# ikt-luh/Unified-Point-Cloud-Compression

Measured on AMD Instinct MI355X. Metric: points/sec encode+decode, longdress vox10, 1 GPU; bpp & D1-PSNR parity, higher is better.
Workload: dtype f32

## Files before the change

### include/pcc_hip.h

```cpp
#ifndef PCC_HIP_H
#define PCC_HIP_H

#include <stddef.h>
#include <stdint.h>

#ifdef __cplusplus
extern "C" {
#endif

#define PCC_OK 0
#define PCC_EINVAL (-1)
#define PCC_EHIP (-2)
#define PCC_EWS (-3)

#define PCC_ACT_NONE 0
#define PCC_ACT_RELU 1
#define PCC_ACT_LEAKY 2

#define PCC_MAP_HDR_INTS 512
#define PCC_MAP_MAX_SEG 8

int pcc_version(void);
const char* pcc_last_error(void);
int pcc_device_info(int* h_cu_count, char* h_arch, int h_arch_len);
// ... 30 lines not shown
int pcc_coords_expand_csr(const int64_t* keys, int64_t n, int32_t kernel_size, int32_t ts_out,
                          const int32_t* h_lattice, int64_t* out_keys, int64_t* d_count, int32_t* pair_ids,
                          int32_t* first, void* ws, size_t ws_bytes, void* stream);

int64_t pcc_map_nbr_elems(int64_t n_out, int32_t kernel_size, int32_t stride, int32_t transposed);
size_t pcc_map_ws_bytes(int64_t n_out);
int pcc_kernel_map_build(const int64_t* in_keys, int64_t n_in, const int64_t* out_keys, int64_t n_out,
                         int32_t kernel_size, int32_t step, int32_t stride, int32_t transposed,
                         int32_t* hdr, int32_t* nbr, int32_t* rows ,
                         int64_t* d_pairs, const uint64_t* grid_bits , const int32_t* grid_rank,
                         const int32_t* h_grid, void* ws, size_t ws_bytes, void* stream);

int64_t pcc_grid_words(const int32_t* h_grid);
size_t pcc_grid_ws_bytes(int64_t words);
int pcc_grid_build(const int64_t* keys, int64_t n, const int32_t* h_grid, uint64_t* bits ,
                   int32_t* rank , void* ws, size_t ws_bytes, void* stream);
int pcc_coords_stride_grid(const int64_t* keys, int64_t n, const int64_t* d_n, const int32_t* h_grid, uint64_t* bits,
                           int32_t* rank, int64_t* out_keys, int64_t* d_count, void* ws, size_t ws_bytes, void* stream);
int pcc_keys_canonicalize_grid(const int64_t* keys, int64_t n, const int32_t* h_grid, uint64_t* bits, int32_t* rank,
                               int64_t* out_keys, int32_t* first_user, int64_t* d_count, void* ws, size_t ws_bytes,
                               void* stream);
int pcc_coords_expand_grid(const int64_t* keys, int64_t n, int32_t kernel_size, const int32_t* h_out, uint64_t* bits,
                           int32_t* rank, int64_t* out_keys, int64_t* d_count, void* ws, size_t ws_bytes, void* stream);
size_t pcc_convt_rows_int_ws_bytes(int64_t pairs, int32_t K);
int64_t pcc_convt_rows_t_elems(int64_t pairs, int32_t K, int32_t cout);
int pcc_convt_fwd_rows(const float* feat_in, int64_t n_in, int32_t cin, const float* packed_w, const float* bias,
                       int32_t K, int32_t cout, const int32_t* first, const int32_t* pair_ids, int64_t n_out,
                       int64_t pairs, float* T, float* out, int32_t act, float slope, void* int_ws, size_t int_ws_bytes,
                       int32_t arith , int32_t* d_guard , void* stream);
int pcc_map_from_csr(const int32_t* first, const int32_t* pair_ids, int64_t n_out, int32_t kernel_size, int32_t* hdr,
                     int32_t* nbr, void* stream);
size_t pcc_expand_grid_csr_ws_bytes(int64_t n_out);
int pcc_coords_expand_grid_csr(const int64_t* out_keys, int64_t n_out, int32_t kernel_size, int32_t ts_out,
                               const uint64_t* in_bits, const int32_t* in_rank, const int32_t* h_in, int64_t n_in,
                               int32_t* first, int32_t* pair_ids, int64_t* d_total, void* ws, size_t ws_bytes, void* stream);
int64_t pcc_expand_grid_csr_slot_elems(int64_t n_out, int32_t kernel_size);
int pcc_coords_expand_grid_csr_slots(const int64_t* out_keys, int64_t n_out, int32_t kernel_size, int32_t ts_out,
                                     const uint64_t* in_bits, const int32_t* in_rank, const int32_t* h_in, int64_t n_in,
                                     int32_t* first, int32_t* pair_ids, int32_t* wg_end, int64_t* d_total , int32_t zk,
                                     void* stream);
int pcc_coords_expand_grid_csr_zk(const int64_t* out_keys, int64_t n_out, int32_t kernel_size, int32_t ts_out,
                               const uint64_t* in_bits, const int32_t* in_rank, const int32_t* h_in, int64_t n_in,
                               int32_t* first, int32_t* pair_ids, int64_t* d_total, void* ws, size_t ws_bytes, void* stream);
int pcc_map_to_dense(const int32_t* hdr, const int32_t* nbr, const int32_t* rows, int64_t n_out,
                     int32_t K, int32_t* dense, void* stream);

// ... 231 lines not shown
```

### unified_point_cloud_compression_amd/csrc/pcc_keys.hip

```cpp
#include <stdarg.h>
#include <stdio.h>
#include <string.h>

#include "pcc_common.h"

static thread_local char g_err[512] = "";

void pcc_set_error(const char* fmt, ...) {
  va_list ap;
  va_start(ap, fmt);
  vsnprintf(g_err, sizeof(g_err), fmt, ap);
  va_end(ap);
}

extern "C" const char* pcc_last_error(void) { return g_err; }
extern "C" int pcc_version(void) { return 100; }

extern "C" int pcc_device_info(int* h_cu_count, char* h_arch, int h_arch_len) {
  int dev = 0;
  PCC_CHECK_HIP(hipGetDevice(&dev));
  hipDeviceProp_t p;
  PCC_CHECK_HIP(hipGetDeviceProperties(&p, dev));
  if (h_cu_count) *h_cu_count = p.multiProcessorCount;
  if (h_arch && h_arch_len > 0) {
// ... 666 lines not shown
    }
  }
#pragma unroll
  for (int c = 0; c < 4; ++c) {
    for (int d = 32; d >= 1; d >>= 1) { mn[c] = min(mn[c], __shfl_xor(mn[c], d)); mx[c] = max(mx[c], __shfl_xor(mx[c], d)); }
    if ((threadIdx.x & 63) == 0) { atomicMin(&s_min[c], mn[c]); atomicMax(&s_max[c], mx[c]); }
  }
  __syncthreads();
  if (threadIdx.x < 4) { atomicMin(&out8[threadIdx.x], s_min[threadIdx.x]); atomicMax(&out8[4 + threadIdx.x], s_max[threadIdx.x]); }
}

extern "C" int pcc_coords_bounds(const void* coords, int32_t is_float, int64_t n, int32_t* out8, void* stream) {
  hipStream_t s = (hipStream_t)stream;
  PCC_REQUIRE(coords && out8 && n >= 1, "pcc_coords_bounds: bad arguments");
  PCC_CHECK_HIP(hipMemsetAsync(out8, 0x7F, 16, s));
  PCC_CHECK_HIP(hipMemsetAsync(out8 + 4, 0x80, 16, s));
  const unsigned g = (unsigned)(pcc_cdiv(n, 256) < 1024 ? pcc_cdiv(n, 256) : 1024);
  if (is_float) k_coords_bounds<float><<<g, 256, 0, s>>>((const float*)coords, n, out8);
  else k_coords_bounds<int><<<g, 256, 0, s>>>((const int*)coords, n, out8);
  PCC_LAUNCH_CHECK();
  return PCC_OK;
}

__device__ __forceinline__ void intake_block_reduce(int (&v)[9], int* __restrict__ part) {
  __shared__ int s_red[4][9];
#pragma unroll
  for (int c = 0; c < 9; ++c) {
    for (int d = 32; d >= 1; d >>= 1) v[c] = min(v[c], __shfl_xor(v[c], d));
    if ((threadIdx.x & 63) == 0) s_red[threadIdx.x >> 6][c] = v[c];
  }
  __syncthreads();
  if (threadIdx.x < 9) {
    const int c = threadIdx.x;
    part[blockIdx.x * 16 + c] = min(min(s_red[0][c], s_red[1][c]), min(s_red[2][c], s_red[3][c]));
  }
}

__global__ void __launch_bounds__(256) k_frame_intake(const float* __restrict__ pc, long long n, long long* __restrict__ keys,
                                                      float4* __restrict__ feats, int* __restrict__ part) {
  int v[9] = {0, 0x7FFFFFFF, 0x7FFFFFFF, 0x7FFFFFFF, 0, 0x7FFFFFFF, 0x7FFFFFFF, 0x7FFFFFFF, 1};
  for (long long i = (long long)blockIdx.x * 256 + threadIdx.x; i < n; i += (long long)gridDim.x * 256) {
    const float2* r = reinterpret_cast<const float2*>(pc + i * 6);
    const float2 a = r[0], b = r[1], c = r[2];
    const int x = (int)floorf(a.x), y = (int)floorf(a.y), z = (int)floorf(b.x);
    const long long k = pack4(0, x, y, z);
    keys[i] = k;
    feats[i] = make_float4(1.f, b.y, c.x, c.y);
    v[1] = min(v[1], x); v[2] = min(v[2], y); v[3] = min(v[3], z);
    v[5] = min(v[5], -x); v[6] = min(v[6], -y); v[7] = min(v[7], -z);
    if (i > 0) {
      const float* q = pc + (i - 1) * 6;
      if (k <= pack4(0, (int)floorf(q[0]), (int)floorf(q[1]), (int)floorf(q[2]))) v[8] = 0;
    }
  }
  intake_block_reduce(v, part);
}

__global__ void __launch_bounds__(256) k_coords_intake_i32(const int4* __restrict__ c4, long long n, long long* __restrict__ keys,
                                                           int* __restrict__ part) {
  int v[9] = {0x7FFFFFFF, 0x7FFFFFFF, 0x7FFFFFFF, 0x7FFFFFFF, 0x7FFFFFFF, 0x7FFFFFFF, 0x7FFFFFFF, 0x7FFFFFFF, 1};
  for (long long i = (long long)blockIdx.x * 256 + threadIdx.x; i < n; i += (long long)gridDim.x * 256) {
    const int4 c = c4[i];
    const long long k = pack4(c.x, c.y, c.z, c.w);
    keys[i] = k;
    v[0] = min(v[0], c.x); v[1] = min(v[1], c.y); v[2] = min(v[2], c.z); v[3] = min(v[3], c.w);
    v[4] = min(v[4], -c.x); v[5] = min(v[5], -c.y); v[6] = min(v[6], -c.z); v[7] = min(v[7], -c.w);
    if (i > 0) {
      const int4 q = c4[i - 1];
      if (k <= pack4(q.x, q.y, q.z, q.w)) v[8] = 0;
    }
  }
  intake_block_reduce(v, part);
}

__global__ void __launch_bounds__(256) k_intake_reduce(const int* __restrict__ part, int nblk, int* __restrict__ out12) {
  __shared__ int s_red[4][9];
  int v[9];
#pragma unroll
  for (int c = 0; c < 9; ++c) v[c] = 0x7FFFFFFF;
  for (int b = threadIdx.x; b < nblk; b += 256)
#pragma unroll
    for (int c = 0; c < 9; ++c) v[c] = min(v[c], part[b * 16 + c]);
#pragma unroll
  for (int c = 0; c < 9; ++c) {
    for (int d = 32; d >= 1; d >>= 1) v[c] = min(v[c], __shfl_xor(v[c], d));
    if ((threadIdx.x & 63) == 0) s_red[threadIdx.x >> 6][c] = v[c];
  }
  __syncthreads();
  if (threadIdx.x < 9) {
    const int c = threadIdx.x;
    out12[c] = min(min(s_red[0][c], s_red[1][c]), min(s_red[2][c], s_red[3][c]));
  }
}

extern "C" size_t pcc_frame_intake_ws_bytes(void) { return (size_t)1024 * 16 * sizeof(int); }

extern "C" int pcc_frame_intake(const float* pc, int64_t n, int64_t* keys, float* feats, int32_t* out12, void* ws, size_t ws_bytes,
                                void* stream) {
  hipStream_t s = (hipStream_t)stream;
  PCC_REQUIRE(pc && keys && feats && out12 && ws && n >= 1, "pcc_frame_intake: bad arguments");
  PCC_REQUIRE((((uintptr_t)pc & 7) | ((uintptr_t)feats & 15)) == 0, "pcc_frame_intake: the frame must be 8-byte, the features 16-byte aligned");
  if (ws_bytes < pcc_frame_intake_ws_bytes()) { pcc_set_error("pcc_frame_intake: workspace too small"); return PCC_EWS; }
  const unsigned g = (unsigned)(pcc_cdiv(n, 256) < 1024 ? pcc_cdiv(n, 256) : 1024);
  k_frame_intake<<<g, 256, 0, s>>>(pc, n, (long long*)keys, (float4*)feats, (int*)ws);
  k_intake_reduce<<<1, 256, 0, s>>>((const int*)ws, (int)g, out12);
  PCC_LAUNCH_CHECK();
  return PCC_OK;
}

extern "C" int pcc_coords_intake_i32(const int32_t* coords, int64_t n, int64_t* keys, int32_t* out12, void* ws, size_t ws_bytes,
                                     void* stream) {
  hipStream_t s = (hipStream_t)stream;
// ... 53 lines not shown
```

### unified_point_cloud_compression_amd/csrc/pcc_map.hip

```cpp
#include <string.h>

#include "pcc_common.h"

struct SegPlan {
  int nseg;
  int K;
  int listed;
  int k_count[PCC_MAP_MAX_SEG];
  int koff_begin[PCC_MAP_MAX_SEG];
  unsigned char koffs[192];
  unsigned char order[192];
};

__device__ __forceinline__ void write_hdr(const SegPlan& plan, const int* __restrict__ class_begin, int class_stride,
                                          int64_t n_out, int* __restrict__ hdr) {
  {
    const int i = (int)threadIdx.x;
    if (i < plan.K && i < 192) {
      hdr[HDR_KOFFS + i] = plan.listed ? plan.koffs[i] : i;
      hdr[HDR_ORDER + i] = plan.order[i];
    }
  }
  if (threadIdx.x != 0) return;
  hdr[HDR_NSEG] = plan.nseg;
// ... 334 lines not shown
  int* class_begin = (int*)p;           p += 1024;
  void* sort_ws = p;
  dim3 g1((unsigned)pcc_cdiv(n_out, 256));
  k_classify<<<g1, 256, 0, s>>>(out_keys, n_out, ilog2(step), stride, cls);
  PCC_LAUNCH_CHECK();
  PCC_TRY(pcc_sort_keys((const int64_t*)cls, n_out, 0xFFull, (int64_t*)cls_sorted, rows, sort_ws,
                        ws_bytes - (size_t)(p - (char*)ws), s));
  k_class_begin<<<1, 64, 0, s>>>(cls_sorted, n_out, nclass, class_begin);
  PCC_LAUNCH_CHECK();
  k_write_hdr<<<1, 192, 0, s>>>(plan, class_begin, 1, n_out, hdr);
  PCC_LAUNCH_CHECK();
  dim3 gdim((unsigned)pcc_cdiv(n_out, 256), (unsigned)max_class_k(kernel_size, stride));
  k_map_transposed<<<gdim, 256, 0, s>>>(grid, in_keys, (int)n_in, out_keys, n_out, kernel_size, step, hdr, rows, nbr,
                                        block_counts);
  PCC_LAUNCH_CHECK();
  if (d_pairs) {
    k_sum_counts<<<1, 1024, 0, s>>>(block_counts, (int64_t)gdim.x * gdim.y, d_pairs);
    PCC_LAUNCH_CHECK();
  }
  return PCC_OK;
}

static int grid_rank(const unsigned long long* b, int64_t words, int32_t* rank, const int32_t* h, int tsl, int64_t* out_keys,
                     int64_t* d_count, void* ws, size_t ws_bytes, hipStream_t s);
__device__ inline long long grid_cell(const int64_t key, const int lo0, const int lo1, const int lo2, const int d0,
                                      const int d1, const int d2, const int tsl) {
  const int b = (int)(key >> 48);
  const int cx = ((int)((key >> 32) & 0xFFFF) - (int)PCC_BIAS - lo0) >> tsl;
  const int cy = ((int)((key >> 16) & 0xFFFF) - (int)PCC_BIAS - lo1) >> tsl;
  const int cz = ((int)(key & 0xFFFF) - (int)PCC_BIAS - lo2) >> tsl;
  return (((long long)b * d0 + cx) * d1 + cy) * d2 + cz;
}

__global__ void k_grid_bits(const int64_t* __restrict__ keys, int64_t n, int lo0, int lo1, int lo2, int d0, int d1,
                            int d2, int tsl, unsigned long long* __restrict__ bits) {
  const int64_t i = (int64_t)blockIdx.x * blockDim.x + threadIdx.x;
  if (i >= n) return;
  const long long c = grid_cell(keys[i], lo0, lo1, lo2, d0, d1, d2, tsl);
  const long long w = c >> 6;
  if (i > 0 && (grid_cell(keys[i - 1], lo0, lo1, lo2, d0, d1, d2, tsl) >> 6) == w) return;
  unsigned long long acc = 1ull << (c & 63);
  for (int64_t t = i + 1; t < n && t < i + 64; ++t) {
    const long long c2 = grid_cell(keys[t], lo0, lo1, lo2, d0, d1, d2, tsl);
    if ((c2 >> 6) != w) break;
    acc |= 1ull << (c2 & 63);
  }
  bits[w] = acc;
// ... 159 lines not shown
    unsigned long long x = bits[wi];
    if (!x) continue;
    int r = rk_s[li];
    long long cell = wi * 64;
    const int z0 = (int)(cell % d2); cell /= d2;
    const int y0 = (int)(cell % d1); cell /= d1;
    const int x0 = (int)(cell % d0);
    const int b0 = (int)(cell / d0);
    while (x) {
      const int bit = __ffsll((long long)x) - 1;
      x &= x - 1;
      int cz = z0 + bit, cy = y0, cx = x0, b = b0;
      while (cz >= d2) {
        cz -= d2;
        if (++cy == d1) { cy = 0; if (++cx == d0) { cx = 0; ++b; } }
      }
      const int64_t X = (int64_t)(lo0 + (cx << tsl)) + PCC_BIAS, Y = (int64_t)(lo1 + (cy << tsl)) + PCC_BIAS,
                    Z = (int64_t)(lo2 + (cz << tsl)) + PCC_BIAS;
      keys[r++] = ((int64_t)b << 48) | (X << 32) | (Y << 16) | Z;
    }
  }
}

static int grid_rank(const unsigned long long* b, int64_t words, int32_t* rank, const int32_t* h, int tsl, int64_t* out_keys,
                     int64_t* d_count, void* ws, size_t ws_bytes, hipStream_t s) {
  const int64_t nb = pcc_cdiv(words, GR_B);
  if (nb <= GR_SELF_NB && (((uintptr_t)b | (uintptr_t)rank) & 15) == 0) {
    if (out_keys) k_grid_rank_apply<true, true><<<(unsigned)nb, 256, 0, s>>>(b, words, nullptr, rank, h[0], h[1], h[2], h[3], h[4], h[5], tsl, out_keys, d_count);
    else k_grid_rank_apply<false, true><<<(unsigned)nb, 256, 0, s>>>(b, words, nullptr, rank, 0, 0, 0, 1, 1, 1, 0, nullptr, nullptr);
    PCC_LAUNCH_CHECK();
    return PCC_OK;
  }
  if (nb <= GR_DIRECT_NB && ws_bytes >= (size_t)nb * 4 + 256 && (((uintptr_t)b | (uintptr_t)rank) & 15) == 0) {
    int* sums = (int*)ws;
    k_grid_rank_reduce<<<(unsigned)nb, 256, 0, s>>>(b, words, sums);
    k_grid_rank_apply<false><<<(unsigned)nb, 256, 0, s>>>(b, words, sums, rank, 0, 0, 0, 1, 1, 1, 0, nullptr, nullptr);
    PCC_LAUNCH_CHECK();
    if (out_keys) {
      k_grid_enumerate<<<(unsigned)pcc_cdiv(words, 256), 256, 0, s>>>(b, rank, words, h[0], h[1], h[2], h[3], h[4], h[5], tsl, out_keys, d_count);
      PCC_LAUNCH_CHECK();
    }
    return PCC_OK;
  }
  k_grid_popc<<<(unsigned)pcc_cdiv(words, 256), 256, 0, s>>>(b, words, rank);
  PCC_LAUNCH_CHECK();
  PCC_TRY(pcc_scan_exclusive_i32(rank, rank, words, ws, ws_bytes, s));
  if (out_keys) {
    k_grid_enumerate<<<(unsigned)pcc_cdiv(words, 256), 256, 0, s>>>(b, rank, words, h[0], h[1], h[2], h[3], h[4], h[5], tsl, out_keys, d_count);
    PCC_LAUNCH_CHECK();
  }
  return PCC_OK;
}

extern "C" int pcc_coords_stride_grid(const int64_t* keys, int64_t n, const int64_t* d_n, const int32_t* h_grid, uint64_t* bits,
                                      int32_t* rank, int64_t* out_keys, int64_t* d_count, void* ws, size_t ws_bytes,
                                      void* stream) {
  hipStream_t s = (hipStream_t)stream;
  PCC_REQUIRE(h_grid && bits && rank && out_keys && d_count, "pcc_coords_stride_grid: NULL array");
// ... 297 lines not shown

__global__ void k_set_int(int* p, int v) { *p = v; }

extern "C" int pcc_coords_expand_grid(const int64_t* keys, int64_t n, int32_t kernel_size, const int32_t* h_out,
                                      uint64_t* bits, int32_t* rank, int64_t* out_keys, int64_t* d_count, void* ws,
                                      size_t ws_bytes, void* stream) {
  hipStream_t s = (hipStream_t)stream;
  PCC_REQUIRE(keys && h_out && bits && rank && out_keys && d_count && n > 0, "pcc_coords_expand_grid: bad arguments");
  PCC_REQUIRE(kernel_size == 2 || kernel_size == 3 || kernel_size == 5, "pcc_coords_expand_grid: kernel_size %d unsupported", kernel_size);
  const int64_t words = pcc_grid_words(h_out);
  PCC_REQUIRE(words >= 1 && words < (1ll << 31), "pcc_coords_expand_grid: lattice too large (%lld words)", (long long)words);
  const int ts_out = h_out[6];
  PCC_REQUIRE(ts_out >= 1 && (ts_out & (ts_out - 1)) == 0, "pcc_coords_expand_grid: pitch must be a power of two");
  if (ws_bytes < pcc_grid_ws_bytes(words)) { pcc_set_error("pcc_coords_expand_grid: workspace too small"); return PCC_EWS; }
  PCC_CHECK_HIP(hipMemsetAsync(bits, 0, (size_t)words * 8, s));
  const dim3 g((unsigned)pcc_cdiv(n, 256), (unsigned)(kernel_size * kernel_size));
  unsigned long long* b = (unsigned long long*)bits;
  const int tsl = ilog2(ts_out);
  if (kernel_size == 2) k_expand_mark<2><<<g, 256, 0, s>>>(keys, n, ts_out, h_out[0], h_out[1], h_out[2], h_out[3], h_out[4], h_out[5], tsl, b);
  else if (kernel_size == 3) k_expand_mark<3><<<g, 256, 0, s>>>(keys, n, ts_out, h_out[0], h_out[1], h_out[2], h_out[3], h_out[4], h_out[5], tsl, b);
  else k_expand_mark<5><<<g, 256, 0, s>>>(keys, n, ts_out, h_out[0], h_out[1], h_out[2], h_out[3], h_out[4], h_out[5], tsl, b);
  PCC_LAUNCH_CHECK();
  return grid_rank(b, words, rank, h_out, tsl, out_keys, d_count, ws, ws_bytes, s);
}

extern "C" size_t pcc_expand_grid_csr_ws_bytes(int64_t n_out) { return pcc_scan_ws_bytes(n_out + 1) + 256; }

static int expand_grid_csr(const int64_t* out_keys, int64_t n_out, int32_t kernel_size, int32_t ts_out,
                           const uint64_t* in_bits, const int32_t* in_rank, const int32_t* h_in,
                           int64_t n_in, int32_t* first, int32_t* pair_ids, int64_t* d_total, void* ws, size_t ws_bytes, int zk,
                           void* stream);
extern "C" int pcc_coords_expand_grid_csr(const int64_t* out_keys, int64_t n_out, int32_t kernel_size, int32_t ts_out,
                                          const uint64_t* in_bits, const int32_t* in_rank, const int32_t* h_in,
                                          int64_t n_in, int32_t* first, int32_t* pair_ids, int64_t* d_total, void* ws,
                                          size_t ws_bytes, void* stream) {
  return expand_grid_csr(out_keys, n_out, kernel_size, ts_out, in_bits, in_rank, h_in, n_in, first, pair_ids, d_total, ws, ws_bytes, 0, stream);
}
extern "C" int pcc_coords_expand_grid_csr_zk(const int64_t* out_keys, int64_t n_out, int32_t kernel_size, int32_t ts_out,
                                             const uint64_t* in_bits, const int32_t* in_rank, const int32_t* h_in,
                                             int64_t n_in, int32_t* first, int32_t* pair_ids, int64_t* d_total, void* ws,
                                             size_t ws_bytes, void* stream) {
  return expand_grid_csr(out_keys, n_out, kernel_size, ts_out, in_bits, in_rank, h_in, n_in, first, pair_ids, d_total, ws, ws_bytes, 1, stream);
}
static int expand_grid_csr(const int64_t* out_keys, int64_t n_out, int32_t kernel_size, int32_t ts_out,
                           const uint64_t* in_bits, const int32_t* in_rank, const int32_t* h_in,
                           int64_t n_in, int32_t* first, int32_t* pair_ids, int64_t* d_total, void* ws, size_t ws_bytes, int zk,
// ... 129 lines not shown
```

### unified_point_cloud_compression_amd/lib.py

```python
import ctypes as C
import os
import threading

import torch

_HERE = os.path.dirname(os.path.abspath(__file__))
LIB_PATH = os.path.join(_HERE, "libpcc_hip.so")

MAP_HDR_INTS = 512
FORM_NAMES = ("other", "k_gemm_h2", "k_gemm_bf2", "k_pair_h2", "pair_bf", "k_conv_mfma_bf", "k_conv_mfma", "k_conv_wave16",
              "k_convt_gather_csr")
MAP_MAX_SEG = 8
ACT_NONE, ACT_RELU, ACT_LEAKY = 0, 1, 2

_p = C.c_void_p
_i32, _i64, _u64, _f32, _sz = C.c_int32, C.c_int64, C.c_uint64, C.c_float, C.c_size_t

SIGNATURES = {
    "pcc_version": (C.c_int, []),
    "pcc_last_error": (C.c_char_p, []),
    "pcc_device_info": (C.c_int, [C.POINTER(C.c_int), C.c_char_p, C.c_int]),
    "pcc_coords_bounds": (C.c_int, [_p, _i32, _i64, _p, _p]),
    "pcc_rows_gather": (C.c_int, [_p, _p, _i64, _i32, _p, _p]),
    "pcc_keys_pack_i32": (C.c_int, [_p, _i64, _p, _p]),
# ... 1 lines not shown
    "pcc_keys_unpack": (C.c_int, [_p, _i64, _p, _p]),
    "pcc_batch_bounds": (C.c_int, [_p, _p, _i64, _i32, _p, _p, _p, _p]),
    "pcc_sort_ws_bytes": (_sz, [_i64]),
    "pcc_sort_keys": (C.c_int, [_p, _i64, _u64, _p, _p, _p, _sz, _p]),
    "pcc_unique_ws_bytes": (_sz, [_i64]),
    "pcc_unique_sorted": (C.c_int, [_p, _i64, _p, _p, _p, _p, _sz, _p]),
    "pcc_keys_is_canonical": (C.c_int, [_p, _i64, _p, _p]),
    "pcc_stride_ws_bytes": (_sz, [_i64]),
    "pcc_coords_stride": (C.c_int, [_p, _i64, _i32, _u64, _p, _p, _p, _sz, _p]),
    "pcc_expand_ws_bytes": (_sz, [_i64, _i32]),
    "pcc_coords_expand": (C.c_int, [_p, _i64, _i32, _i32, _u64, _p, _p, _p, _sz, _p]),
    "pcc_expand_csr_ws_bytes": (_sz, [_i64, _i32]),
    "pcc_coords_expand_csr": (C.c_int, [_p, _i64, _i32, _i32, C.POINTER(_i32), _p, _p, _p, _p, _p, _sz, _p]),
    "pcc_map_nbr_elems": (_i64, [_i64, _i32, _i32, _i32]),
    "pcc_map_ws_bytes": (_sz, [_i64]),
    "pcc_kernel_map_build": (C.c_int, [_p, _i64, _p, _i64, _i32, _i32, _i32, _i32, _p, _p, _p, _p, _p, _p,
                                       C.POINTER(_i32), _p, _sz, _p]),
    "pcc_grid_words": (_i64, [C.POINTER(_i32)]),
    "pcc_grid_ws_bytes": (_sz, [_i64]),
    "pcc_grid_build": (C.c_int, [_p, _i64, C.POINTER(_i32), _p, _p, _p, _sz, _p]),
    "pcc_coords_stride_grid": (C.c_int, [_p, _i64, _p, _p, _p, _p, _p, _p, _p, _sz, _p]),
    "pcc_keys_canonicalize_grid": (C.c_int, [_p, _i64, _p, _p, _p, _p, _p, _p, _p, _sz, _p]),
    "pcc_coords_expand_grid": (C.c_int, [_p, _i64, _i32, _p, _p, _p, _p, _p, _p, _sz, _p]),
    "pcc_expand_grid_csr_ws_bytes": (_sz, [_i64]),
    "pcc_coords_expand_grid_csr": (C.c_int, [_p, _i64, _i32, _i32, _p, _p, _p, _i64, _p, _p, _p, _p, _sz, _p]),
    "pcc_coords_expand_grid_csr_zk": (C.c_int, [_p, _i64, _i32, _i32, _p, _p, _p, _i64, _p, _p, _p, _p, _sz, _p]),
    "pcc_expand_grid_csr_slot_elems": (_i64, [_i64, _i32]),
    "pcc_coords_expand_grid_csr_slots": (C.c_int, [_p, _i64, _i32, _i32, _p, _p, _p, _i64, _p, _p, _p, _p, _i32, _p]),
    "pcc_map_to_dense": (C.c_int, [_p, _p, _p, _i64, _i32, _p, _p]),
    "pcc_set_in4_min_rows": (C.c_int, [_i64]),
    "pcc_set_thin_z_min_rows": (C.c_int, [_i64]),
    "pcc_conv_packed_elems": (_i64, [_i32, _i32, _i32]),
    "pcc_conv_pack_weights": (C.c_int, [_p, _i32, _i32, _i32, _p, _i64, _p]),
    "pcc_conv_pack_weights_ex": (C.c_int, [_p, _i32, _i32, _i32, _i32, _i32, _p, _i64, _p]),
    "pcc_conv_ws_bytes": (_sz, [_i64, _i32, _i32, _i32]),
    "pcc_conv_fwd": (C.c_int, [_p, _i64, _i32, _p, _p, _i32, _i32, _p, _p, _p, _i64, _p, _i32, _f32, _p, _sz, _i32, _p, _p]),
    "pcc_conv_head_supported": (C.c_int, [_i32, _i32]),
    "pcc_conv_head_ws_bytes": (_sz, [_i64]),
    "pcc_conv_head_fwd": (C.c_int, [_p, _i64, _i32, _p, _p, _i32, _p, _p, _p, _p, _p, _p, _p, _p, _sz, _p]),
    "pcc_band_tiles_cap": (_i64, [_i64, _i32, _i32]),
    "pcc_band_tiles_ws_bytes": (_sz, [_i32, _i32]),
    "pcc_band_tiles_build": (C.c_int, [_p, _i64, _i32, _i32, _i32, _i32, _i32, _i32, _p, _i64, _p, _p, _sz, _p]),
    "pcc_convt_packed_elems": (_i64, [_i32, _i32, _i32]),
    "pcc_convt_pack_weights": (C.c_int, [_p, _i32, _i32, _i32, _p, _i64, _p]),
    "pcc_convt_fwd": (C.c_int, [_p, _i64, _i32, _p, _p, _i32, _i32, _p, _p, _p, _i64, _p, _p, _i32, _f32, _i32, _p, _p]),
    "pcc_convt_fwd_csr": (C.c_int, [_p, _i64, _i32, _p, _p, _i32, _i32, _p, _p, _i64, _p, _p, _i32, _f32, _p, _i32, _p,
# ... 266 lines not shown
```

### unified_point_cloud_compression_amd/model/transforms.py

```python

import torch
import torch.nn as nn

from .. import MinkowskiEngine as ME
from .. import lib as L
from .. import sparse as S
from ..MinkowskiEngine.sparse_tensor import SparseTensor
from .blocks import MinkowskiGDN


def batch_segments(cset):
    return batch_segments_many([cset])[0]


def batch_segments_begin(cs):
    if cs.bounds.bmax == 0 or "segments" in cs._derived or cs.bounds.bmax > 10 or cs.n == 0:
        return None
    entries = cs.bounds.bmax + 2
    a, b, c = L.counter(4), L.counter(4), L.counter(4)
    L.call("pcc_batch_bounds", L.ptr(cs.keys), None, cs.n, entries, L.cptr(a), L.cptr(b), L.cptr(c), L.stream())

    def finish(v):
        cs._derived["segments"] = [int(x) for x in (list(v[0]) + list(v[1]) + list(v[2]))[:entries]]
        return cs._derived["segments"]
# ... 219 lines not shown
        csr7 = cs_in.csr_for(out_set.keys, out_set.n, 7, ts_out, zk=True, slots=from_grid)
        if from_grid:
            h = S.convt_forward_csr_grid(feats, packedM, c0.bias, 343, gen.in_channels, c0.out_channels, csr7, out_set,
                                         L.ACT_RELU, cb)
            w2 = c2._packed.get(c2.kernel, state_dict_order=True)
            logit = S.conv_thin_grid_forward(h, w2, c2.bias, c0.out_channels, c2.out_channels, out_set)
        else:
            kmap3 = out_set.kernel_map(out_set, 3)
            h = S.convt_forward_csr(feats, packedM, c0.bias, 343, gen.in_channels, c0.out_channels, csr7, out_set.n,
                                    act=L.ACT_RELU, ex_map=kmap3, ex_bias=cb)
            logit = c2._apply_conv(SparseTensor._from_canonical(out_set, h), out_set, kmap3)
        pred = SparseTensor._from_canonical(out_set, logit)
        if probe is None:
            seg, bids = batch_segments(out_set)
            ks = [int(k_lvl[b]) if (seg[i + 1] > seg[i]) else 0 for i, b in enumerate(bids)]
            mask, keys, n = S.topk_prune_keys(logit, seg, ks, out_set.keys)
        else:
            mask, n_keep = self._topk_prediction(pred, k_lvl)
            forced = probe("select", lvl, out_set, logit, mask, None)
            if forced is not None:
                mask, n_keep = forced, int(forced.sum().item())
            keys, _, n = S.prune(out_set.keys, out_set.n, None, mask, n_keep)
        kept = S.CoordSet(keys, n, ts_out, out_set.bounds)
        if "_packed_conv" not in gen.__dict__:
            gen.__dict__["_packed_conv"] = S.PackedConv(transposed=False)
        packed = gen._packed_conv.get(gen.kernel, state_dict_order=True)
        rows_form = bool(L.load().pcc_conv_pairs_supported(125, gen.in_channels, gen.out_channels))
        total = L.counter() if rows_form else None
        csr5 = cs_in.csr_for(kept.keys, n, 5, ts_out, total=total)
        nxt = None
        if next_up is not None and n > 0:
            g2 = next_up[-1]
            if isinstance(g2, ME.MinkowskiGenerativeConvolutionTranspose) and ts_out % g2.stride == 0:
                nxt = kept.expand_begin(g2.kernel_size, ts_out // g2.stride, want_csr=False)
        pairs = S.resolve(S.Pending(total, lambda v: int(v[0])) if rows_form else None, nxt)[0]
        if rows_form:
            xk = S.convt_forward_rows(feats, packed, gen.bias, 125, gen.in_channels, gen.out_channels, csr5, n, pairs_bound=pairs)
        else:
            xk = S.conv_forward(feats, packed, gen.bias, 125, gen.in_channels, gen.out_channels,
                                S.map_from_csr(csr5, cs_in.n, n, 5), n)
        if probe is not None:
            probe("kept", lvl, kept, None, None, xk)
        return SparseTensor._from_canonical(kept, xk), pred, mask

    def forward(self, y, coords=None, k=None, trace=None, probe=None):
        predictions = []
# ... 31 lines not shown
```

### unified_point_cloud_compression_amd/sparse.py

```python
import ctypes as C

import itertools
import weakref

import torch

from . import lib as L

BIAS = 1 << 15


def _field_mask(lo, hi):
    a, b = lo + BIAS, hi + BIAS
    return (1 << (a ^ b).bit_length()) - 1


class Bounds:

    def __init__(self, bmax, lo, hi):
        self.bmax, self.lo, self.hi = int(bmax), tuple(int(v) for v in lo), tuple(int(v) for v in hi)
        if min(self.lo) < -BIAS + 64 or max(self.hi) >= BIAS - 64 or self.bmax >= (1 << 15):
            raise L.PccError(f"coordinates out of the 16-bit key range: lo={self.lo} hi={self.hi} batch={self.bmax}")

    def bit_mask(self):
# ... 52 lines not shown
        return self._plan_pending

    def pair_plan(self):
        if not hasattr(self, "_plan"):
            resolve(self.pair_plan_begin())
        return self._plan

    def dense(self):
        out = torch.empty((self.K, self.n_out), dtype=torch.int32, device=self.hdr.device)
        if self.n_out:
            L.call("pcc_map_to_dense", L.ptr(self.hdr), L.ptr(self.nbr), L.ptr(self.rows), self.n_out, self.K,
                   L.ptr(out), L.stream())
        return out


PAIR_MIN_K = 64
PAIR_MAX_DENSITY = 0.5
PAIR_MIN_CIN = 64
COUNT_PAIRS = False
MORTON_MIN_ROWS = 1 << 62
USE_CSR = True
CANON_BY_GRID = True
EXPAND_BY_GRID = True
STRIDE_BY_GRID = True
USE_GRID = True
GRID_MAX_BYTES = 8 << 30
BAND_TILES = True
BAND_MIN_ROWS = 1 << 20
BAND_COUNT = 16
HEAD_FUSED = True


_SET_SERIAL = itertools.count()


class Pending:

    __slots__ = ("counter", "finish", "result", "done", "keys_out", "cap")

    def __init__(self, counter, finish):
        self.counter, self.finish, self.result, self.done = counter, finish, None, False


def resolve(*pendings):
    todo = [p for p in pendings if p is not None and not p.done]
    if todo:
# ... 191 lines not shown
    def _expand_by_grid(self, ksize, ts_out):
        K = ksize ** 3
        _, _, _, words = self._expand_lattice(ksize, ts_out)
        if (USE_CSR and USE_GRID and EXPAND_BY_GRID and self.n > 0 and ksize in (2, 3, 5) and words < (1 << 31)
                and words * 12 <= GRID_MAX_BYTES and self.n * K < (1 << 31)):
            return self.grid()
        return None

    def expand_begin(self, ksize, ts_out, want_csr=True):
        key = ("expand", ksize, ts_out)
        if key in self._derived:
            return _ready(self.expand(ksize, ts_out, want_csr))
        if not self._expand_by_grid(ksize, ts_out):
            return None
        dev = self.device
        lib = L.load()
        ob, cells, h, words = self._expand_lattice(ksize, ts_out)
        m = self.n * ksize ** 3
        bits = torch.empty(words, dtype=torch.int64, device=dev)
        rank = torch.empty(words, dtype=torch.int32, device=dev)
        out = torch.empty(min(m, cells), dtype=torch.int64, device=dev)
        cnt = L.counter()
        ws = L.workspace(lib.pcc_grid_ws_bytes(words), dev)
        L.call("pcc_coords_expand_grid", L.ptr(self.keys), self.n, ksize, h, L.ptr(bits), L.ptr(rank), L.ptr(out),
               L.cptr(cnt), L.ptr(ws), ws.numel(), L.stream())
        entries = ob.bmax + 2 if 0 < ob.bmax <= 10 else 0
        if entries:
            seg_a, seg_b, seg_c = L.counter(4), L.counter(4), L.counter(4)
            L.call("pcc_batch_bounds", L.ptr(out), L.cptr(cnt), 0, entries, L.cptr(seg_a), L.cptr(seg_b), L.cptr(seg_c), L.stream())

        def finish(v):
            segs = None
            if v and isinstance(v[0], (list, tuple)):
                segs = (list(v[1]) + list(v[2]) + list(v[3]))[:entries]
                v = v[0]
            n = int(v[0])
            cs = CoordSet(out[:n].clone() if n < out.numel() // 2 else out, n, ts_out, ob)
            cs._grid = (bits, rank, h)
            cs._on_lattice = self._on_lattice
            if segs is not None:
                cs._derived["segments"] = [int(x) for x in segs]
            self._derived[key] = cs
            if want_csr:
                self._derived[("csr", ksize, ts_out)] = self.csr_for(cs.keys, n, ksize, ts_out)
            return cs
        if ksize == 2 and self.ts == 2 * ts_out and self._on_lattice:
            return _ready(finish([8 * self.n]))
        return Pending([cnt, seg_a, seg_b, seg_c] if entries else cnt, finish)
# ... 118 lines not shown
        self._pcc_chain = chain


def frame_intake(pc):
    n = pc.shape[0]
    keys = torch.empty(n, dtype=torch.int64, device=pc.device)
    feats = torch.empty((n, 4), dtype=torch.float32, device=pc.device)
    out = torch.empty(12, dtype=torch.int32, device=pc.device)
    ws = L.workspace(L.load().pcc_frame_intake_ws_bytes(), pc.device)
    L.call("pcc_frame_intake", L.ptr(pc), n, L.ptr(keys), L.ptr(feats), L.ptr(out), L.ptr(ws), ws.numel(), L.stream())
    v = out.tolist()
    return keys, feats, Bounds(0, v[1:4], [-x for x in v[5:8]]), bool(v[8])


def coords_intake(coords):
    n = coords.shape[0]
    keys = torch.empty(n, dtype=torch.int64, device=coords.device)
    out = torch.empty(12, dtype=torch.int32, device=coords.device)
    ws = L.workspace(L.load().pcc_frame_intake_ws_bytes(), coords.device)
    L.call("pcc_coords_intake_i32", L.ptr(coords), n, L.ptr(keys), L.ptr(out), L.ptr(ws), ws.numel(), L.stream())
    v = out.tolist()
    if v[0] < 0:
        raise L.PccError("negative batch index")
    return keys, Bounds(-v[4], v[1:4], [-x for x in v[5:8]]), bool(v[8])


def coordset_from_coords(coords, tensor_stride, stride_chain=None):
    n = coords.shape[0]
    stride_chain = getattr(coords, "_pcc_chain", stride_chain)
    hint = getattr(coords, "_pcc_hint", None)
    if hint is not None:
        keys, b, canonical = hint[:3]
    elif n > 1 and coords.dtype == torch.int32 and coords.is_contiguous() and coords.data_ptr() % 16 == 0:
        keys, b, canonical = coords_intake(coords)
    else:
        keys = pack_keys(coords)
        b, canonical = bounds_of(coords, canon_keys=keys if n > 1 else None) if n > 1 else (bounds_of(coords), True)
    if n <= 1 or canonical:
        cs = CoordSet(keys, n, tensor_stride, b)
        if stride_chain and n > 1:
            resolve(cs.stride_chain_begin(stride_chain))
        return cs, None, None
    dev = coords.device
    lib = L.load()
    dims = [(b.hi[i] - b.lo[i]) // tensor_stride + 1 for i in range(3)]
    h = (C.c_int32 * 8)(b.lo[0], b.lo[1], b.lo[2], dims[0], dims[1], dims[2], tensor_stride, b.bmax + 1)
    words = lib.pcc_grid_words(h)
    on_lattice = all(v % tensor_stride == 0 for v in b.lo)
    if USE_GRID and CANON_BY_GRID and on_lattice and words < (1 << 31) and words * 12 <= GRID_MAX_BYTES:
        bits = torch.empty(words, dtype=torch.int64, device=dev)
        rank = torch.empty(words, dtype=torch.int32, device=dev)
        ukeys = torch.empty(n, dtype=torch.int64, device=dev)
        first_user = torch.empty(n, dtype=torch.int32, device=dev)
        cnt = L.counter(2)
        ws = L.workspace(lib.pcc_grid_ws_bytes(words), dev)
        L.call("pcc_keys_canonicalize_grid", L.ptr(keys), n, h, L.ptr(bits), L.ptr(rank), L.ptr(ukeys), L.ptr(first_user),
               L.cptr(cnt), L.ptr(ws), ws.numel(), L.stream())
        cs = CoordSet(ukeys, n, tensor_stride, b)
        chain = cs.stride_chain_begin(stride_chain, keys=keys, n_keys=n) if stride_chain else None
        (nu, off_lattice), _ = resolve(Pending(cnt, lambda v: (int(v[0]), int(v[1]))), chain)
        if not off_lattice:
            cs.n = nu
# ... 396 lines not shown
```

Before: 54.60 million.

## Expand coordinates by gathering parent occupancy bitgrid instead of scattering keys

Adds a gather-style expand kernel. Each output bitgrid word is computed from the parent lattice's occupancy bits through bit-spreading and dilation, replacing the scatter of each input key's kernel neighbourhood. The kernel also produces per-block popcounts, so grid_rank can skip its reduce pass. Intake kernels now compute the coordinate pitch (common trailing zero bits), which is used to mark coord sets as on-lattice so the gather path qualifies. This adds bit-manipulation complexity and precondition checks on lattice alignment.

```diff
diff --git a/include/pcc_hip.h b/include/pcc_hip.h
--- a/include/pcc_hip.h
+++ b/include/pcc_hip.h
@@ -76,6 +76,9 @@
                                void* stream);
 int pcc_coords_expand_grid(const int64_t* keys, int64_t n, int32_t kernel_size, const int32_t* h_out, uint64_t* bits,
                            int32_t* rank, int64_t* out_keys, int64_t* d_count, void* ws, size_t ws_bytes, void* stream);
+int pcc_coords_expand_grid_gather(const uint64_t* in_bits, const int32_t* h_in, int32_t kernel_size, const int32_t* h_out,
+                                  uint64_t* bits, int32_t* rank, int64_t* out_keys, int64_t* d_count, void* ws,
+                                  size_t ws_bytes, void* stream);
 size_t pcc_convt_rows_int_ws_bytes(int64_t pairs, int32_t K);
 int64_t pcc_convt_rows_t_elems(int64_t pairs, int32_t K, int32_t cout);
 int pcc_convt_fwd_rows(const float* feat_in, int64_t n_in, int32_t cin, const float* packed_w, const float* bias,
diff --git a/unified_point_cloud_compression_amd/csrc/pcc_keys.hip b/unified_point_cloud_compression_amd/csrc/pcc_keys.hip
--- a/unified_point_cloud_compression_amd/csrc/pcc_keys.hip
+++ b/unified_point_cloud_compression_amd/csrc/pcc_keys.hip
@@ -712,15 +712,15 @@
   return PCC_OK;
 }
 
-__device__ __forceinline__ void intake_block_reduce(int (&v)[9], int* __restrict__ part) {
-  __shared__ int s_red[4][9];
-#pragma unroll
-  for (int c = 0; c < 9; ++c) {
+__device__ __forceinline__ void intake_block_reduce(int (&v)[10], int* __restrict__ part) {
+  __shared__ int s_red[4][10];
+#pragma unroll
+  for (int c = 0; c < 10; ++c) {
     for (int d = 32; d >= 1; d >>= 1) v[c] = min(v[c], __shfl_xor(v[c], d));
     if ((threadIdx.x & 63) == 0) s_red[threadIdx.x >> 6][c] = v[c];
   }
   __syncthreads();
-  if (threadIdx.x < 9) {
+  if (threadIdx.x < 10) {
     const int c = threadIdx.x;
     part[blockIdx.x * 16 + c] = min(min(s_red[0][c], s_red[1][c]), min(s_red[2][c], s_red[3][c]));
   }
@@ -728,7 +728,7 @@
 
 __global__ void __launch_bounds__(256) k_frame_intake(const float* __restrict__ pc, long long n, long long* __restrict__ keys,
                                                       float4* __restrict__ feats, int* __restrict__ part) {
-  int v[9] = {0, 0x7FFFFFFF, 0x7FFFFFFF, 0x7FFFFFFF, 0, 0x7FFFFFFF, 0x7FFFFFFF, 0x7FFFFFFF, 1};
+  int v[10] = {0, 0x7FFFFFFF, 0x7FFFFFFF, 0x7FFFFFFF, 0, 0x7FFFFFFF, 0x7FFFFFFF, 0x7FFFFFFF, 1, 31};
   for (long long i = (long long)blockIdx.x * 256 + threadIdx.x; i < n; i += (long long)gridDim.x * 256) {
     const float2* r = reinterpret_cast<const float2*>(pc + i * 6);
     const float2 a = r[0], b = r[1], c = r[2];
@@ -738,6 +738,7 @@
     feats[i] = make_float4(1.f, b.y, c.x, c.y);
     v[1] = min(v[1], x); v[2] = min(v[2], y); v[3] = min(v[3], z);
     v[5] = min(v[5], -x); v[6] = min(v[6], -y); v[7] = min(v[7], -z);
+    v[9] = min(v[9], __ffs((x | y | z) | (int)0x80000000) - 1);
     if (i > 0) {
       const float* q = pc + (i - 1) * 6;
       if (k <= pack4(0, (int)floorf(q[0]), (int)floorf(q[1]), (int)floorf(q[2]))) v[8] = 0;
@@ -748,13 +749,14 @@
 
 __global__ void __launch_bounds__(256) k_coords_intake_i32(const int4* __restrict__ c4, long long n, long long* __restrict__ keys,
                                                            int* __restrict__ part) {
-  int v[9] = {0x7FFFFFFF, 0x7FFFFFFF, 0x7FFFFFFF, 0x7FFFFFFF, 0x7FFFFFFF, 0x7FFFFFFF, 0x7FFFFFFF, 0x7FFFFFFF, 1};
+  int v[10] = {0x7FFFFFFF, 0x7FFFFFFF, 0x7FFFFFFF, 0x7FFFFFFF, 0x7FFFFFFF, 0x7FFFFFFF, 0x7FFFFFFF, 0x7FFFFFFF, 1, 31};
   for (long long i = (long long)blockIdx.x * 256 + threadIdx.x; i < n; i += (long long)gridDim.x * 256) {
     const int4 c = c4[i];
     const long long k = pack4(c.x, c.y, c.z, c.w);
     keys[i] = k;
     v[0] = min(v[0], c.x); v[1] = min(v[1], c.y); v[2] = min(v[2], c.z); v[3] = min(v[3], c.w);
     v[4] = min(v[4], -c.x); v[5] = min(v[5], -c.y); v[6] = min(v[6], -c.z); v[7] = min(v[7], -c.w);
+    v[9] = min(v[9], __ffs((c.y | c.z | c.w) | (int)0x80000000) - 1);
     if (i > 0) {
       const int4 q = c4[i - 1];
       if (k <= pack4(q.x, q.y, q.z, q.w)) v[8] = 0;
@@ -764,20 +766,20 @@
 }
 
 __global__ void __launch_bounds__(256) k_intake_reduce(const int* __restrict__ part, int nblk, int* __restrict__ out12) {
-  __shared__ int s_red[4][9];
-  int v[9];
-#pragma unroll
-  for (int c = 0; c < 9; ++c) v[c] = 0x7FFFFFFF;
+  __shared__ int s_red[4][10];
+  int v[10];
+#pragma unroll
+  for (int c = 0; c < 10; ++c) v[c] = 0x7FFFFFFF;
   for (int b = threadIdx.x; b < nblk; b += 256)
 #pragma unroll
-    for (int c = 0; c < 9; ++c) v[c] = min(v[c], part[b * 16 + c]);
-#pragma unroll
-  for (int c = 0; c < 9; ++c) {
+    for (int c = 0; c < 10; ++c) v[c] = min(v[c], part[b * 16 + c]);
+#pragma unroll
+  for (int c = 0; c < 10; ++c) {
     for (int d = 32; d >= 1; d >>= 1) v[c] = min(v[c], __shfl_xor(v[c], d));
     if ((threadIdx.x & 63) == 0) s_red[threadIdx.x >> 6][c] = v[c];
   }
   __syncthreads();
-  if (threadIdx.x < 9) {
+  if (threadIdx.x < 10) {
     const int c = threadIdx.x;
     out12[c] = min(min(s_red[0][c], s_red[1][c]), min(s_red[2][c], s_red[3][c]));
   }
diff --git a/unified_point_cloud_compression_amd/csrc/pcc_map.hip b/unified_point_cloud_compression_amd/csrc/pcc_map.hip
--- a/unified_point_cloud_compression_amd/csrc/pcc_map.hip
+++ b/unified_point_cloud_compression_amd/csrc/pcc_map.hip
@@ -380,7 +380,7 @@
 }
 
 static int grid_rank(const unsigned long long* b, int64_t words, int32_t* rank, const int32_t* h, int tsl, int64_t* out_keys,
-                     int64_t* d_count, void* ws, size_t ws_bytes, hipStream_t s);
+                     int64_t* d_count, void* ws, size_t ws_bytes, hipStream_t s, bool have_sums = false);
 __device__ inline long long grid_cell(const int64_t key, const int lo0, const int lo1, const int lo2, const int d0,
                                       const int d1, const int d2, const int tsl) {
   const int b = (int)(key >> 48);
@@ -586,8 +586,13 @@
   }
 }
 
+static bool grid_rank_takes_sums(const void* b, const void* rank, int64_t words, size_t ws_bytes) {
+  const int64_t nb = pcc_cdiv(words, GR_B);
+  return nb > GR_SELF_NB && nb <= GR_DIRECT_NB && ws_bytes >= (size_t)nb * 4 + 256 && (((uintptr_t)b | (uintptr_t)rank) & 15) == 0;
+}
+
 static int grid_rank(const unsigned long long* b, int64_t words, int32_t* rank, const int32_t* h, int tsl, int64_t* out_keys,
-                     int64_t* d_count, void* ws, size_t ws_bytes, hipStream_t s) {
+                     int64_t* d_count, void* ws, size_t ws_bytes, hipStream_t s, bool have_sums) {
   const int64_t nb = pcc_cdiv(words, GR_B);
   if (nb <= GR_SELF_NB && (((uintptr_t)b | (uintptr_t)rank) & 15) == 0) {
     if (out_keys) k_grid_rank_apply<true, true><<<(unsigned)nb, 256, 0, s>>>(b, words, nullptr, rank, h[0], h[1], h[2], h[3], h[4], h[5], tsl, out_keys, d_count);
@@ -597,7 +602,7 @@
   }
   if (nb <= GR_DIRECT_NB && ws_bytes >= (size_t)nb * 4 + 256 && (((uintptr_t)b | (uintptr_t)rank) & 15) == 0) {
     int* sums = (int*)ws;
-    k_grid_rank_reduce<<<(unsigned)nb, 256, 0, s>>>(b, words, sums);
+    if (!have_sums) k_grid_rank_reduce<<<(unsigned)nb, 256, 0, s>>>(b, words, sums);
     k_grid_rank_apply<false><<<(unsigned)nb, 256, 0, s>>>(b, words, sums, rank, 0, 0, 0, 1, 1, 1, 0, nullptr, nullptr);
     PCC_LAUNCH_CHECK();
     if (out_keys) {
@@ -941,6 +946,153 @@
   else k_expand_mark<5><<<g, 256, 0, s>>>(keys, n, ts_out, h_out[0], h_out[1], h_out[2], h_out[3], h_out[4], h_out[5], tsl, b);
   PCC_LAUNCH_CHECK();
   return grid_rank(b, words, rank, h_out, tsl, out_keys, d_count, ws, ws_bytes, s);
+}
+
+struct ExpandGatherArgs {
+  const unsigned long long* in_bits; int in_words;
+  int D0, D1, D2;
+  int d0, d1, d2, nbatch;
+  int du0, du1, du2;
+  long long words;
+  unsigned long long* bits;
+  int* sums;
+};
+
+__device__ __forceinline__ unsigned long long spread_even(unsigned long long x) {
+  x &= 0xFFFFFFFFull;
+  x = (x | (x << 16)) & 0x0000FFFF0000FFFFull;
+  x = (x | (x << 8)) & 0x00FF00FF00FF00FFull;
+  x = (x | (x << 4)) & 0x0F0F0F0F0F0F0F0Full;
+  x = (x | (x << 2)) & 0x3333333333333333ull;
+  x = (x | (x << 1)) & 0x5555555555555555ull;
+  return x;
+}
+
+template <int KS>
+__device__ __forceinline__ unsigned long long gather_segment(const ExpandGatherArgs& a, int b, int x, int y, int z, int L) {
+  constexpr int H = (KS - 1) / 2, NC = H + 1;
+  const int ux = x + a.du0, uy = y + a.du1, uz = z + a.du2;
+  int X0 = (ux - H + 1) >> 1, X1 = (ux + H) >> 1, Y0 = (uy - H + 1) >> 1, Y1 = (uy + H) >> 1;
+  int Z0 = (uz - H + 1) >> 1, Z1 = (uz + L - 1 + H) >> 1;
+  X0 = X0 < 0 ? 0 : X0; Y0 = Y0 < 0 ? 0 : Y0; Z0 = Z0 < 0 ? 0 : Z0;
+  X1 = X1 >= a.D0 ? a.D0 - 1 : X1; Y1 = Y1 >= a.D1 ? a.D1 - 1 : Y1; Z1 = Z1 >= a.D2 ? a.D2 - 1 : Z1;
+  const int nz = Z1 - Z0 + 1;
+  const bool any = X1 >= X0 && Y1 >= Y0 && nz > 0;
+  const int c00 = any ? ((b * a.D0 + X0) * a.D1 + Y0) * a.D2 + Z0 : 0;
+  const int slab = a.D1 * a.D2;
+  unsigned long long w0[NC * NC], w1[NC * NC];
+  int sh[NC * NC];
+#pragma unroll
+  for (int jx = 0; jx < NC; ++jx)
+#pragma unroll
+    for (int jy = 0; jy < NC; ++jy) {
+      const bool ok = X0 + jx <= X1 && Y0 + jy <= Y1;
+      const int c = c00 + (ok ? jx * slab + jy * a.D2 : 0);
+      const int wi = c >> 6;
+      sh[jx * NC + jy] = ok ? (c & 63) : 64;
+      w0[jx * NC + jy] = a.in_bits[wi];
+      w1[jx * NC + jy] = a.in_bits[wi + 1 < a.in_words ? wi + 1 : wi];
+    }
+  unsigned long long P = 0;
+#pragma unroll
+  for (int j = 0; j < NC * NC; ++j) {
+    const int s = sh[j];
+    unsigned long long f = s < 64 ? w0[j] >> s : 0ull;
+    if (s > 0 && s < 64) f |= w1[j] << (64 - s);
+    P |= f;
+  }
+  if (!any) return 0ull;
+  P &= (1ull << nz) - 1ull;
+  if (!P) return 0ull;
+  const int o0 = 2 * Z0 - uz + H;
+  unsigned __int128 T = ((unsigned __int128)spread_even(P >> 32) << 64) | spread_even(P);
+  T <<= o0;
+  unsigned __int128 M = T;
+#pragma unroll
+  for (int d = 1; d <= H; ++d) M |= (T << d) | (T >> d);
+  const unsigned long long r = (unsigned long long)(M >> H);
+  return L < 64 ? r & ((1ull << L) - 1ull) : r;
+}
+
+struct GatherWalk { int b, x, y, z; };
+
+template <int KS>
+__device__ __forceinline__ unsigned long long gather_word(const ExpandGatherArgs& a, GatherWalk& p) {
+  unsigned long long acc = 0;
+  int bit = 0;
+  while (bit < 64 && p.b < a.nbatch) {
+    const int left = a.d2 - p.z;
+    const int L = left < 64 - bit ? left : 64 - bit;
+    acc |= gather_segment<KS>(a, p.b, p.x, p.y, p.z, L) << bit;
+    bit += L;
+    p.z += L;
+    if (p.z == a.d2) { p.z = 0; if (++p.y == a.d1) { p.y = 0; if (++p.x == a.d0) { p.x = 0; ++p.b; } } }
+  }
+  return acc;
+}
+
+template <int KS>
+__global__ void __launch_bounds__(256) k_expand_mark_gather(ExpandGatherArgs a) {
+  __shared__ int wsum[4];
+  const long long base = (long long)blockIdx.x * GR_B + (long long)threadIdx.x * 8;
+  int c = 0;
+  if (base < a.words) {
+    GatherWalk p;
+    long long cell = base * 64;
+    p.z = (int)(cell % a.d2); cell /= a.d2;
+    p.y = (int)(cell % a.d1); cell /= a.d1;
+    p.x = (int)(cell % a.d0); cell /= a.d0;
+    p.b = cell < a.nbatch ? (int)cell : a.nbatch;
+    const bool full = base + 8 <= a.words;
+#pragma unroll 1
+    for (int q = 0; q < 8; q += 2) {
+      if (!full && base + q >= a.words) break;
+      const unsigned long long v0 = gather_word<KS>(a, p);
+      const unsigned long long v1 = gather_word<KS>(a, p);
+      c += __popcll(v0) + __popcll(v1);
+      *reinterpret_cast<ulonglong2*>(a.bits + base + q) = make_ulonglong2(v0, v1);
+    }
+  }
+  if (!a.sums) return;
+#pragma unroll
+  for (int d = 32; d >= 1; d >>= 1) c += __shfl_xor(c, d);
+  if ((threadIdx.x & 63) == 0) wsum[threadIdx.x >> 6] = c;
+  __syncthreads();
+  if (threadIdx.x == 0) a.sums[blockIdx.x] = wsum[0] + wsum[1] + wsum[2] + wsum[3];
+}
+
+extern "C" int pcc_coords_expand_grid_gather(const uint64_t* in_bits, const int32_t* h_in, int32_t kernel_size,
+                                             const int32_t* h_out, uint64_t* bits, int32_t* rank, int64_t* out_keys,
+                                             int64_t* d_count, void* ws, size_t ws_bytes, void* stream) {
+  hipStream_t s = (hipStream_t)stream;
+  PCC_REQUIRE(in_bits && h_in && h_out && bits && rank && out_keys && d_count, "pcc_coords_expand_grid_gather: bad arguments");
+  PCC_REQUIRE(kernel_size == 3 || kernel_size == 5, "pcc_coords_expand_grid_gather: kernel_size %d unsupported (odd kernels 3 and 5)", kernel_size);
+  const int ts_out = h_out[6];
+  PCC_REQUIRE(ts_out >= 1 && (ts_out & (ts_out - 1)) == 0, "pcc_coords_expand_grid_gather: pitch must be a power of two");
+  PCC_REQUIRE(h_in[6] == 2 * ts_out, "pcc_coords_expand_grid_gather: the parent pitch %d must be twice the output pitch %d", h_in[6], ts_out);
+  PCC_REQUIRE(h_in[7] == h_out[7] && h_in[7] >= 1, "pcc_coords_expand_grid_gather: parent and output lattice differ in their batch count");
+  for (int ax = 0; ax < 3; ++ax) {
+    PCC_REQUIRE(h_in[3 + ax] >= 1 && h_out[3 + ax] >= 1, "pcc_coords_expand_grid_gather: empty lattice");
+    PCC_REQUIRE((h_out[ax] - h_in[ax]) % ts_out == 0, "pcc_coords_expand_grid_gather: the lattice origins differ by %d, no multiple of the output pitch %d", h_out[ax] - h_in[ax], ts_out);
+  }
+  const int64_t words = pcc_grid_words(h_out), in_words = pcc_grid_words(h_in);
+  PCC_REQUIRE(words >= 1 && words < (1ll << 31), "pcc_coords_expand_grid_gather: lattice too large (%lld words)", (long long)words);
+  PCC_REQUIRE(in_words >= 1 && in_words <= (1ll << 25), "pcc_coords_expand_grid_gather: parent lattice too large (%lld words)", (long long)in_words);
+  PCC_REQUIRE(((uintptr_t)bits & 15) == 0, "pcc_coords_expand_grid_gather: bits must be 16-byte aligned");
+  if (ws_bytes < pcc_grid_ws_bytes(words)) { pcc_set_error("pcc_coords_expand_grid_gather: workspace too small"); return PCC_EWS; }
+  unsigned long long* b = (unsigned long long*)bits;
+  const bool sums = grid_rank_takes_sums(b, rank, words, ws_bytes);
+  ExpandGatherArgs a;
+  a.in_bits = (const unsigned long long*)in_bits; a.in_words = (int)in_words;
+  a.D0 = h_in[3]; a.D1 = h_in[4]; a.D2 = h_in[5];
+  a.d0 = h_out[3]; a.d1 = h_out[4]; a.d2 = h_out[5]; a.nbatch = h_out[7];
+  a.du0 = (h_out[0] - h_in[0]) / ts_out; a.du1 = (h_out[1] - h_in[1]) / ts_out; a.du2 = (h_out[2] - h_in[2]) / ts_out;
+  a.words = words; a.bits = b; a.sums = sums ? (int*)ws : nullptr;
+  const unsigned g = (unsigned)pcc_cdiv(words, GR_B);
+  if (kernel_size == 3) k_expand_mark_gather<3><<<g, 256, 0, s>>>(a);
+  else k_expand_mark_gather<5><<<g, 256, 0, s>>>(a);
+  PCC_LAUNCH_CHECK();
+  return grid_rank(b, words, rank, h_out, ilog2(ts_out), out_keys, d_count, ws, ws_bytes, s, sums);
 }
 
 extern "C" size_t pcc_expand_grid_csr_ws_bytes(int64_t n_out) { return pcc_scan_ws_bytes(n_out + 1) + 256; }
diff --git a/unified_point_cloud_compression_amd/lib.py b/unified_point_cloud_compression_amd/lib.py
--- a/unified_point_cloud_compression_amd/lib.py
+++ b/unified_point_cloud_compression_amd/lib.py
@@ -47,6 +47,7 @@
     "pcc_coords_stride_grid": (C.c_int, [_p, _i64, _p, _p, _p, _p, _p, _p, _p, _sz, _p]),
     "pcc_keys_canonicalize_grid": (C.c_int, [_p, _i64, _p, _p, _p, _p, _p, _p, _p, _sz, _p]),
     "pcc_coords_expand_grid": (C.c_int, [_p, _i64, _i32, _p, _p, _p, _p, _p, _p, _sz, _p]),
+    "pcc_coords_expand_grid_gather": (C.c_int, [_p, _p, _i32, _p, _p, _p, _p, _p, _p, _sz, _p]),
     "pcc_expand_grid_csr_ws_bytes": (_sz, [_i64]),
     "pcc_coords_expand_grid_csr": (C.c_int, [_p, _i64, _i32, _i32, _p, _p, _p, _i64, _p, _p, _p, _p, _sz, _p]),
     "pcc_coords_expand_grid_csr_zk": (C.c_int, [_p, _i64, _i32, _i32, _p, _p, _p, _i64, _p, _p, _p, _p, _sz, _p]),
diff --git a/unified_point_cloud_compression_amd/model/transforms.py b/unified_point_cloud_compression_amd/model/transforms.py
--- a/unified_point_cloud_compression_amd/model/transforms.py
+++ b/unified_point_cloud_compression_amd/model/transforms.py
@@ -265,6 +265,7 @@
                 mask, n_keep = forced, int(forced.sum().item())
             keys, _, n = S.prune(out_set.keys, out_set.n, None, mask, n_keep)
         kept = S.CoordSet(keys, n, ts_out, out_set.bounds)
+        kept._on_lattice = out_set._on_lattice
         if "_packed_conv" not in gen.__dict__:
             gen.__dict__["_packed_conv"] = S.PackedConv(transposed=False)
         packed = gen._packed_conv.get(gen.kernel, state_dict_order=True)
diff --git a/unified_point_cloud_compression_amd/sparse.py b/unified_point_cloud_compression_amd/sparse.py
--- a/unified_point_cloud_compression_amd/sparse.py
+++ b/unified_point_cloud_compression_amd/sparse.py
@@ -98,6 +98,7 @@
 USE_CSR = True
 CANON_BY_GRID = True
 EXPAND_BY_GRID = True
+EXPAND_GATHER = True
 STRIDE_BY_GRID = True
 USE_GRID = True
 GRID_MAX_BYTES = 8 << 30
@@ -335,8 +336,14 @@
         out = torch.empty(min(m, cells), dtype=torch.int64, device=dev)
         cnt = L.counter()
         ws = L.workspace(lib.pcc_grid_ws_bytes(words), dev)
-        L.call("pcc_coords_expand_grid", L.ptr(self.keys), self.n, ksize, h, L.ptr(bits), L.ptr(rank), L.ptr(out),
-               L.cptr(cnt), L.ptr(ws), ws.numel(), L.stream())
+        g = self._grid
+        if EXPAND_GATHER and ksize in (3, 5) and self.ts == 2 * ts_out and g and self._on_lattice \
+                and g[0].numel() <= (1 << 25) and all(v % self.ts == 0 for v in g[2][0:3]):
+            L.call("pcc_coords_expand_grid_gather", L.ptr(g[0]), g[2], ksize, h, L.ptr(bits), L.ptr(rank), L.ptr(out),
+                   L.cptr(cnt), L.ptr(ws), ws.numel(), L.stream())
+        else:
+            L.call("pcc_coords_expand_grid", L.ptr(self.keys), self.n, ksize, h, L.ptr(bits), L.ptr(rank), L.ptr(out),
+                   L.cptr(cnt), L.ptr(ws), ws.numel(), L.stream())
         entries = ob.bmax + 2 if 0 < ob.bmax <= 10 else 0
         if entries:
             seg_a, seg_b, seg_c = L.counter(4), L.counter(4), L.counter(4)
@@ -501,22 +508,24 @@
     v = out.tolist()
     if v[0] < 0:
         raise L.PccError("negative batch index")
-    return keys, Bounds(-v[4], v[1:4], [-x for x in v[5:8]]), bool(v[8])
+    return keys, Bounds(-v[4], v[1:4], [-x for x in v[5:8]]), bool(v[8]), 1 << v[9]
 
 
 def coordset_from_coords(coords, tensor_stride, stride_chain=None):
     n = coords.shape[0]
     stride_chain = getattr(coords, "_pcc_chain", stride_chain)
     hint = getattr(coords, "_pcc_hint", None)
+    pitch = 1
     if hint is not None:
         keys, b, canonical = hint[:3]
     elif n > 1 and coords.dtype == torch.int32 and coords.is_contiguous() and coords.data_ptr() % 16 == 0:
-        keys, b, canonical = coords_intake(coords)
+        keys, b, canonical, pitch = coords_intake(coords)
     else:
         keys = pack_keys(coords)
         b, canonical = bounds_of(coords, canon_keys=keys if n > 1 else None) if n > 1 else (bounds_of(coords), True)
     if n <= 1 or canonical:
         cs = CoordSet(keys, n, tensor_stride, b)
+        cs._on_lattice = pitch % tensor_stride == 0
         if stride_chain and n > 1:
             resolve(cs.stride_chain_begin(stride_chain))
         return cs, None, None
```

Measured after the change: 54.97 million (median of 5 runs). Within noise of the previous version (+0.7%).
